# DylanAuty/ObjCAViT

Hardware: AMD Instinct MI355X
Metric: images/sec (640x480, bs=16) forward depth inference, 3 batches of 16 in flight per GPU; AbsRel vs CPU ref (higher is better)
Workload: dtype f32 (fp16 / bf16 split contractions)

## Files before the change

### include/objcavit_hip.h

```cpp
#ifndef OBJCAVIT_HIP_H
#define OBJCAVIT_HIP_H

#include <stddef.h>
#include <stdint.h>

#ifdef __cplusplus
extern "C" {
#endif

typedef void* ocv_stream_t;

#define OCV_ABI_VERSION 5
int ocv_abi_version(void);
const char* ocv_last_error(void);

int ocv_range_flag_set(unsigned* flag);
int ocv_range_flag_take_fwd(unsigned* flag, unsigned* out, ocv_stream_t stream);
int ocv_attention_set_fp32_range(int on);
int ocv_attention_set_dispatch(int form);

#define OCV_ACT_NONE 0
#define OCV_ACT_RELU 1
#define OCV_ACT_LEAKY_RELU 2
#define OCV_ACT_SILU 3
// ... 147 lines not shown
                                    int C, int H, int W, int k, int stride, int pad_t, int pad_l, int Ho, int Wo,
                                    ocv_stream_t stream);
int ocv_se_gate_partials_fwd(const float* part, int tiles, long pixels_per_image, const float* w1, const float* b1,
                             const float* w2t, const float* b2, float* gate, float* hidden_ws, int B, int C, int R,
                             ocv_stream_t stream);
int ocv_depthwise_conv_nhwc_sum_hl_fwd(const float* in, const float* w, const float* bias, float* out, void* out_hl, float* part,
                                       int B, int C, int H, int W, int k, int stride, int pad_t, int pad_l, int Ho, int Wo,
                                       ocv_stream_t stream);
int ocv_se_gate_weights_fwd(const float* part, int tiles, long pixels_per_image, const float* w1, const float* b1,
                            const float* w2t, const float* b2, const float* W, void* w_packed, long w_image_elems, float* gate,
                            float* hidden_ws, int B, int C, int R, int N, ocv_stream_t stream);


size_t ocv_channel_mean_workspace_bytes(int B, int C, long P);
int ocv_channel_mean_nhwc_fwd(const float* x, float* out, int B, int C, long P, void* workspace, size_t workspace_bytes,
                              ocv_stream_t stream);

int ocv_se_gate_fwd(const float* mean, const float* w1, const float* b1, const float* w2t, const float* b2, float* gate,
                    float* hidden_ws, int B, int C, int R, ocv_stream_t stream);

int ocv_conv_nhwc_fwd(const float* x1, int C1, const float* x2, int C2, const void* w_hi, const void* w_lo,
                      const float* bias, const float* residual, float* y, int B, int H, int W, int Cout, int ksize,
                      int act, ocv_stream_t stream);
int ocv_conv_nhwc_exact_fwd(const float* x1, int C1, const float* x2, int C2, const float* w_tap_major, const float* bias,
                            const float* residual, float* y, int B, int H, int W, int Cout, int ksize, int act,
                            ocv_stream_t stream);
int ocv_conv3x3_nhwc_strided_fwd(const float* x, int Cin, const void* w_hi, const void* w_lo, const float* bias,
                                 const float* residual, float* y, int B, int H, int W, int Cout, int stride, int pad_t,
                                 int pad_l, int Ho, int Wo, int act, ocv_stream_t stream);

int ocv_mbconv_expand_dw_tiles(int Ho, int Wo, int k, int stride);
int ocv_mbconv_expand_dw_fwd(const float* x, const void* w_packed, const float* bias_expand, const float* w_dw,
                             const float* bias_dw, float* y, float* part, int B, int H, int W, int Cin, int mid, int k,
                             int stride, int pad_t, int pad_l, int Ho, int Wo, ocv_stream_t stream);

size_t ocv_split_act_elems(int B, int H, int W, int C);

int ocv_conv_nhwc_split_fwd(const void* x_hl, int Cin, const void* w_hi, const void* w_lo, const float* bias,
                            const float* residual, float* y, void* y_hl, int B, int H, int W, int Cout, int ksize,
                            int act, ocv_stream_t stream);
size_t ocv_conv_nhwc_split_workspace_bytes(int B, int H, int W, int Cin, int Cout, int ksize);
int ocv_conv_nhwc_split_ws_fwd(const void* x_hl, int Cin, const void* w_hi, const void* w_lo, const float* bias,
                               const float* residual, float* y, void* y_hl, int B, int H, int W, int Cout, int ksize,
                               int act, void* workspace, size_t workspace_bytes, ocv_stream_t stream);
int ocv_conv_nhwc_split_x_fwd(const void* x_hl, int Cin, const void* w_hi, const void* w_lo, const float* oscale, int f16,
                              const float* bias, const float* residual, float* y, void* y_hl, int B, int H, int W, int Cout,
                              int ksize, int act, void* workspace, size_t workspace_bytes, ocv_stream_t stream);

int ocv_conv3x3_packed_taps_k(int Cin);
int ocv_conv3x3_split_packed_taps_fwd(const void* x_hl, int Cin, const void* w_hi, const void* w_lo, const float* oscale, int f16,
                                      const float* bias, const float* residual, float* y, void* y_hl, int B, int H, int W, int Cout,
                                      int act, ocv_stream_t stream);

size_t ocv_conv3x3_winograd43_workspace_bytes(int B, int H, int W, int Cin, int Cout);
int ocv_conv3x3_winograd43_split_fwd(const void* x_hl, int Cin, const void* u_hi, const void* u_lo, const float* fscale,
                                     const float* cscale, const float* bias, float* y, void* y_hl, int B, int H, int W, int Cout,
                                     int act, int hl_f16, void* workspace, size_t workspace_bytes, ocv_stream_t stream);

int ocv_tap_interp_supported(int h, int w, int H, int W, int Cout);
int ocv_tap_interp_staging_rounds(int h, int w, int H, int W);
int ocv_tap_interp_combine_fwd(const float* z, int h, int w, int zpad, const float* zborder, const float* s, const float* bias,
                               float* y, void* y_hl, int B, int H, int W, int Cout, int act, ocv_stream_t stream);
int ocv_tap_interp_combine_x_fwd(const float* z, int h, int w, int zpad, const float* zborder, const float* s, const float* bias,
                                 float* y, void* y_hl, int hl_f16, int B, int H, int W, int Cout, int act, ocv_stream_t stream);


int ocv_upsample_concat_split_fwd(const float* x, int h, int w, int C1, const float* skip, int C2, void* out_hl, int B,
                                  int H, int W, ocv_stream_t stream);
int ocv_upsample_concat_split_x_fwd(const float* x, int h, int w, int C1, const float* skip, int C2, void* out_hl, int f16, int B,
                                    int H, int W, ocv_stream_t stream);

size_t ocv_depth_metrics_workspace_bytes(int B, int H, int W);
int ocv_depth_metrics_fwd(const float* pred, const float* pred_mirror, int h, int w, const float* gt, int H, int W,
                          float min_depth, float max_depth, int crop_y0, int crop_y1, int crop_x0, int crop_x1,
                          long first_image_id, float* records, int B, void* workspace, size_t workspace_bytes,
                          ocv_stream_t stream);
size_t ocv_depth_metrics_loss_workspace_bytes(int B, int H, int W, int n_bins);
int ocv_depth_metrics_loss_fwd(const float* pred, const float* pred_mirror, int h, int w, const float* gt, int H, int W,
                               float min_depth, float max_depth, int crop_y0, int crop_y1, int crop_x0, int crop_x1,
                               const float* bin_edges, int n_bins, long first_image_id, float* records, float* loss_records, int B,
                               void* workspace, size_t workspace_bytes, ocv_stream_t stream);

int ocv_frame_ingest_fwd(const uint8_t* frames, long frame_stride, long row_stride, int Hs, int Ws, int top, int left,
                         const float* table, float* out, int B, int H, int W, int mirror_too, long mirror_offset,
                         ocv_stream_t stream);
int ocv_depth_ingest_fwd(const uint16_t* depth, long frame_stride, long row_stride, int Hs, int Ws, int top, int left, float factor,
                         float* out, int B, int H, int W, ocv_stream_t stream);
int ocv_depth_finalize_fwd(const float* pred, const float* pred_mirror, int h, int w, float min_depth, float max_depth, int H, int W,
                           float* depth, uint16_t* depth_u16, float u16_scale, uint8_t* rgb8, const uint8_t* colormap, float vmin,
                           float colormap_scale, int B, ocv_stream_t stream);
int ocv_depth_finalize_stats_fwd(const float* pred, const float* pred_mirror, const float* var, const float* var_mirror,
                                 const float* pmax, const float* pmax_mirror, int h, int w, float min_depth, float max_depth, int H, int W,
                                 float* depth_std, float* confidence, int B, ocv_stream_t stream);
int ocv_object_depth_fwd(const float* depth, const float* depth_std, const float* xywh, long xywh_row_stride, const int* counts, int B,
                         int cap, int H, int W, float half, const double* quantiles, int Q, float* out, ocv_stream_t stream);
#define OCV_UNPROJECT_TILE 2048
size_t ocv_depth_unproject_workspace_bytes(int B, int H, int W, int sy, int sx);
int ocv_depth_unproject_fwd(const float* depth, const float* K, const float* confidence, const float* depth_std, const uint8_t* frames,
                            long frame_stride, long row_stride, int Hs, int Ws, int top, int left, int B, int H, int W, int sy, int sx,
                            float near, float far, float min_confidence, float max_std, int cap, float* points, int* pixel, int* counts,
                            int* total, void* workspace, size_t workspace_bytes, ocv_stream_t stream);

#define OCV_BINNORM_LINEAR 0
#define OCV_BINNORM_SIGMOID 1
#define OCV_BINNORM_NONE 2
int ocv_bin_edges_fwd(const float* raw, int mode, float min_depth, float max_depth, float* widths_normed, float* edges,
// ... 23 lines not shown
```

### objcavit_amd/_lib.py

```python
from __future__ import annotations

import ctypes as C
import os
from typing import Optional

_HERE = os.path.dirname(os.path.abspath(__file__))
LIB_PATH = os.environ.get("OCV_LIB_PATH") or os.path.join(_HERE, "lib", "libobjcavit_hip.so")

_f32p = C.c_void_p
_u8p = C.c_void_p
_stream = C.c_void_p
ABI_VERSION = 5


class EncoderLayerParams(C.Structure):
    _fields_ = [("struct_size", C.c_size_t)] + [(n, C.c_void_p) for n in (
        "in_proj_w", "in_proj_b", "out_proj_w", "out_proj_b", "norm1_w", "norm1_b",
        "linear1_w", "linear1_b", "linear2_w", "linear2_b", "norm2_w", "norm2_b",
        "in_proj_p3", "out_proj_p3", "linear1_p3", "linear2_p3",
        "in_proj_h2", "out_proj_h2", "linear1_h2", "linear2_h2")]

    def __init__(self, *a, **kw):
        super().__init__(*a, **kw)
        self.struct_size = C.sizeof(EncoderLayerParams)
# ... 84 lines not shown
    "ocv_depth_metrics_workspace_bytes": (C.c_size_t, [C.c_int] * 3),
    "ocv_depth_metrics_fwd": (C.c_int, [_f32p, _f32p, C.c_int, C.c_int, _f32p, C.c_int, C.c_int, C.c_float, C.c_float] + [C.c_int] * 4 +
                              [C.c_long, _f32p, C.c_int, C.c_void_p, C.c_size_t, _stream]),
    "ocv_depth_metrics_loss_workspace_bytes": (C.c_size_t, [C.c_int] * 4),
    "ocv_depth_metrics_loss_fwd": (C.c_int, [_f32p, _f32p, C.c_int, C.c_int, _f32p, C.c_int, C.c_int, C.c_float, C.c_float] + [C.c_int] * 4 +
                                   [_f32p, C.c_int, C.c_long, _f32p, _f32p, C.c_int, C.c_void_p, C.c_size_t, _stream]),
    "ocv_frame_ingest_fwd": (C.c_int, [_u8p, C.c_long, C.c_long, C.c_int, C.c_int, C.c_int, C.c_int, _f32p, _f32p, C.c_int, C.c_int, C.c_int,
                                       C.c_int, C.c_long, _stream]),
    "ocv_depth_ingest_fwd": (C.c_int, [C.c_void_p, C.c_long, C.c_long, C.c_int, C.c_int, C.c_int, C.c_int, C.c_float, _f32p, C.c_int, C.c_int,
                                       C.c_int, _stream]),
    "ocv_depth_finalize_fwd": (C.c_int, [_f32p, _f32p, C.c_int, C.c_int, C.c_float, C.c_float, C.c_int, C.c_int, _f32p, C.c_void_p, C.c_float,
                                         _u8p, _u8p, C.c_float, C.c_float, C.c_int, _stream]),
    "ocv_depth_finalize_stats_fwd": (C.c_int, [_f32p] * 6 + [C.c_int, C.c_int, C.c_float, C.c_float, C.c_int, C.c_int, _f32p, _f32p, C.c_int,
                                               _stream]),
    "ocv_object_depth_fwd": (C.c_int, [_f32p, _f32p, _f32p, C.c_long, C.c_void_p, C.c_int, C.c_int, C.c_int, C.c_int, C.c_float,
                                       C.POINTER(C.c_double), C.c_int, _f32p, _stream]),
    "ocv_depth_unproject_workspace_bytes": (C.c_size_t, [C.c_int] * 5),
    "ocv_depth_unproject_fwd": (C.c_int, [_f32p, _f32p, _f32p, _f32p, _u8p, C.c_long, C.c_long] + [C.c_int] * 9 + [C.c_float] * 4 +
                                [C.c_int, _f32p, C.c_void_p, C.c_void_p, C.c_void_p, C.c_void_p, C.c_size_t, _stream]),
    "ocv_conv3x3_few_channels_fwd": (C.c_int, [_f32p, C.c_long, C.c_long, C.c_long, C.c_long, _f32p, _f32p] + [C.c_int] * 5 + [_stream]),
    "ocv_stem_conv_fwd": (C.c_int, [_f32p, _f32p, _f32p, _f32p] + [C.c_int] * 12 + [_stream]),
    "ocv_pointwise_packed_weight_elems": (C.c_size_t, [C.c_int, C.c_int]),
    "ocv_pointwise_split_set_dispatch": (C.c_int, [C.c_int, C.c_int, C.c_int]),
    "ocv_pointwise_conv_nhwc_split_fwd": (C.c_int, [_f32p, _f32p, C.c_int, C.c_void_p, _f32p, _f32p, _f32p,
                                                    C.c_long, C.c_int, C.c_int, C.c_int, C.c_void_p]),
    "ocv_pointwise_conv_nhwc_fwd": (C.c_int, [_f32p, _f32p, C.c_int, _f32p, _f32p, _f32p, _f32p, C.c_long, C.c_int, C.c_int,
                                              C.c_int, _stream]),
    "ocv_depthwise_conv_nhwc_fwd": (C.c_int, [_f32p, _f32p, _f32p, _f32p] + [C.c_int] * 11 + [_stream]),
    "ocv_channel_mean_workspace_bytes": (C.c_size_t, [C.c_int, C.c_int, C.c_long]),
    "ocv_channel_mean_nhwc_fwd": (C.c_int, [_f32p, _f32p, C.c_int, C.c_int, C.c_long, C.c_void_p, C.c_size_t, _stream]),
    "ocv_se_gate_fwd": (C.c_int, [_f32p] * 7 + [C.c_int] * 3 + [_stream]),
    "ocv_conv_nhwc_fwd": (C.c_int, [_f32p, C.c_int, _f32p, C.c_int, C.c_void_p, C.c_void_p, _f32p, _f32p, _f32p] +
                          [C.c_int] * 6 + [_stream]),
    "ocv_conv3x3_nhwc_strided_fwd": (C.c_int, [_f32p, C.c_int, C.c_void_p, C.c_void_p, _f32p, _f32p, _f32p] + [C.c_int] * 10 + [_stream]),
    "ocv_conv_nhwc_exact_fwd": (C.c_int, [_f32p, C.c_int, _f32p, C.c_int, _f32p, _f32p, _f32p, _f32p] + [C.c_int] * 6 + [_stream]),
    "ocv_mbconv_expand_dw_tiles": (C.c_int, [C.c_int] * 4),
    "ocv_mbconv_expand_dw_fwd": (C.c_int, [_f32p, C.c_void_p, _f32p, _f32p, _f32p, _f32p, _f32p] + [C.c_int] * 11 + [_stream]),
    "ocv_regressor_bins_fwd": (C.c_int, [_f32p, C.c_long, _f32p, _f32p, _f32p, _f32p, _f32p, _f32p, C.c_int, C.c_int, C.c_int, C.c_int, C.c_float,
                                         C.c_int, C.c_float, C.c_float, _f32p, _f32p, _f32p, C.c_int, _stream]),
    "ocv_bin_edges_fwd": (C.c_int, [_f32p, C.c_int, C.c_float, C.c_float, _f32p, _f32p, _f32p, C.c_int, C.c_int, _stream]),
    "ocv_object_tokens_pad_fwd": (C.c_int, [_f32p, C.c_void_p, C.c_float, _f32p, _u8p, C.c_int, C.c_int, C.c_int, _stream]),
    "ocv_object_front_pad_fwd": (C.c_int, [_f32p, C.c_void_p, C.c_int, C.c_int, C.c_float, _f32p, _u8p] + [C.c_int] * 4 + [_stream]),
    "ocv_split_act_elems": (C.c_size_t, [C.c_int] * 4),
    "ocv_conv_nhwc_split_fwd": (C.c_int, [C.c_void_p, C.c_int, C.c_void_p, C.c_void_p, _f32p, _f32p, _f32p, C.c_void_p]
                                + [C.c_int] * 6 + [_stream]),
    "ocv_conv_nhwc_split_workspace_bytes": (C.c_size_t, [C.c_int] * 6),
    "ocv_conv_nhwc_split_ws_fwd": (C.c_int, [C.c_void_p, C.c_int, C.c_void_p, C.c_void_p, _f32p, _f32p, _f32p, C.c_void_p]
                                   + [C.c_int] * 6 + [C.c_void_p, C.c_size_t, _stream]),
    "ocv_conv_nhwc_split_x_fwd": (C.c_int, [C.c_void_p, C.c_int, C.c_void_p, C.c_void_p, _f32p, C.c_int, _f32p, _f32p, _f32p, C.c_void_p]
                                  + [C.c_int] * 6 + [C.c_void_p, C.c_size_t, _stream]),
    "ocv_conv3x3_packed_taps_k": (C.c_int, [C.c_int]),
    "ocv_conv3x3_split_packed_taps_fwd": (C.c_int, [C.c_void_p, C.c_int, C.c_void_p, C.c_void_p, _f32p, C.c_int, _f32p, _f32p, _f32p, C.c_void_p]
                                          + [C.c_int] * 5 + [_stream]),
    "ocv_upsample_concat_split_x_fwd": (C.c_int, [_f32p, C.c_int, C.c_int, C.c_int, _f32p, C.c_int, C.c_void_p, C.c_int,
                                                  C.c_int, C.c_int, C.c_int, _stream]),
    "ocv_tap_interp_combine_x_fwd": (C.c_int, [_f32p, C.c_int, C.c_int, C.c_int, _f32p, _f32p, _f32p, _f32p, C.c_void_p] + [C.c_int] * 6 + [_stream]),
    "ocv_pos_grid_sample_fwd": (C.c_int, [_f32p, C.c_int, C.c_int, C.c_int, _f32p, C.c_int, C.c_int, C.c_int, C.c_float, C.c_float,
                                          C.c_int, _f32p, _f32p, _stream]),
    "ocv_conv3x3_winograd43_workspace_bytes": (C.c_size_t, [C.c_int] * 5),
    "ocv_conv3x3_winograd43_split_fwd": (C.c_int, [C.c_void_p, C.c_int, C.c_void_p, C.c_void_p, _f32p, _f32p, _f32p, _f32p, C.c_void_p] + [C.c_int] * 6 +
                                         [C.c_void_p, C.c_size_t, _stream]),
    "ocv_tap_interp_supported": (C.c_int, [C.c_int] * 5),
    "ocv_tap_interp_staging_rounds": (C.c_int, [C.c_int] * 4),
    "ocv_tap_interp_combine_fwd": (C.c_int, [_f32p, C.c_int, C.c_int, C.c_int, _f32p, _f32p, _f32p, _f32p, C.c_void_p] + [C.c_int] * 5 + [_stream]),
    "ocv_upsample_concat_split_fwd": (C.c_int, [_f32p, C.c_int, C.c_int, C.c_int, _f32p, C.c_int, C.c_void_p,
                                                C.c_int, C.c_int, C.c_int, _stream]),
}

_lib: Optional[C.CDLL] = None


class HipLibraryError(RuntimeError):
    pass


def load(path: Optional[str] = None) -> C.CDLL:
    global _lib
    if _lib is not None and path is None:
        return _lib
    import torch
    p = path or LIB_PATH
    if not os.path.exists(p):
        raise HipLibraryError(
            f"{p} not found: build it with `python -m objcavit_amd.build` (hipcc --offload-arch=gfx950). "
            "There is no CPU fallback for the ObjCAViT hot path.")
    try:
        lib = C.CDLL(p, mode=C.RTLD_GLOBAL)
    except OSError as e:
        raise HipLibraryError(f"cannot load {p}: {e}") from e
    for name, (res, args) in PROTOTYPES.items():
        try:
            fn = getattr(lib, name)
        except AttributeError as e:
            raise HipLibraryError(f"{p} does not export {name}") from e
        fn.restype = res
        fn.argtypes = args
    if lib.ocv_abi_version() != ABI_VERSION:
        raise HipLibraryError(f"ABI version mismatch: library {lib.ocv_abi_version()}, binding {ABI_VERSION}")
    if path is None:
        _lib = lib
    return lib


def check(rc: int, what: str) -> None:
    if rc != 0:
        msg = load().ocv_last_error().decode(errors="replace")
# ... 2 lines not shown
```

### objcavit_amd/build.py

```python
from __future__ import annotations

import os
import shutil
import subprocess
import sys

HERE = os.path.dirname(os.path.abspath(__file__))
CSRC = os.environ.get("OCV_CSRC_DIR") or os.path.join(HERE, "csrc")
LIB_DIR = os.path.join(HERE, "lib")
LIB_PATH = os.path.join(LIB_DIR, "libobjcavit_hip.so")
SOURCES = ("capi.hip", "linear.hip", "attention.hip", "patch_embed.hip", "bin_head.hip", "depthwise.hip", "conv_igemm.hip", "encoder_nhwc.hip", "upsample.hip", "pointwise_split.hip", "stem.hip", "depthwise_se.hip", "metrics.hip", "mbconv_fused.hip", "pos_sample.hip", "conv_exact.hip", "token_split3.hip", "tap_interp.hip", "pointwise_hl.hip", "xattn_h2.hip", "conv_few.hip", "token_h2.hip", "objects_pad.hip", "bin_edges.hip", "frame_ingest.hip", "depth_finalize.hip", "object_depth.hip", "point_cloud.hip")
ARCH = "gfx950"


def _hipcc() -> str:
    for c in (os.environ.get("HIPCC"), shutil.which("hipcc"), "/opt/rocm/bin/hipcc"):
        if c and os.path.exists(c):
            return c
    raise RuntimeError("hipcc not found")


def _stale() -> bool:
    if not os.path.exists(LIB_PATH):
        return True
    t = os.path.getmtime(LIB_PATH)
    deps = [os.path.join(CSRC, f) for f in os.listdir(CSRC)] + [os.path.join(HERE, "..", "include", "objcavit_hip.h")]
    return any(os.path.getmtime(d) > t for d in deps)


def build(force: bool = False, verbose: bool = False, out: str = None) -> str:
    out = out or os.environ.get("OCV_LIB_OUT")
    if out:
        return _build_to(os.path.abspath(out), os.path.abspath(out) + ".objs", verbose)
    if not force and not _stale():
        return LIB_PATH
    return _build_to(LIB_PATH, LIB_DIR, verbose)


def _build_to(lib_path: str, obj_dir: str, verbose: bool) -> str:
    os.makedirs(os.path.dirname(lib_path), exist_ok=True)
    os.makedirs(obj_dir, exist_ok=True)
    if os.path.exists(lib_path):
        os.remove(lib_path)
    objs = []
    procs = []
    for src in SOURCES:
        obj = os.path.join(obj_dir, src.replace(".hip", ".o"))
        cmd = [_hipcc(), f"--offload-arch={ARCH}", "-O3", "-std=c++17", "-fPIC", "-ffp-contract=fast", "-c",
               os.path.join(CSRC, src), "-o", obj] + os.environ.get("OCV_EXTRA_HIPCC_FLAGS", "").split()
        if verbose:
            cmd.insert(1, "-Rpass-analysis=kernel-resource-usage")
        procs.append((src, subprocess.Popen(cmd, stdout=subprocess.PIPE, stderr=subprocess.STDOUT, text=True)))
        objs.append(obj)
    for src, pr in procs:
        out, _ = pr.communicate()
        if pr.returncode != 0:
            raise RuntimeError(f"hipcc failed on {src}:\n{out}")
        if verbose:
            print(out)
    link = [_hipcc(), f"--offload-arch={ARCH}", "-shared", "-fPIC", "-o", lib_path] + objs
    r = subprocess.run(link, stdout=subprocess.PIPE, stderr=subprocess.STDOUT, text=True)
    if r.returncode != 0:
        raise RuntimeError(f"link failed:\n{r.stdout}")
    for o in objs:
# ... 9 lines not shown
```

### objcavit_amd/csrc/common.hpp

```cpp
#pragma once
#include <hip/hip_runtime.h>
#include <stdint.h>

typedef float f32x16 __attribute__((ext_vector_type(16)));
typedef float f32x4 __attribute__((ext_vector_type(4)));

#define OCV_WAVE 64

__device__ __forceinline__ f32x16 mfma_32x32x2(float a, float b, f32x16 c) {
  return __builtin_amdgcn_mfma_f32_32x32x2f32(a, b, c, 0, 0, 0);
}

__device__ __forceinline__ constexpr int acc_row(int r, int hh) { return (r & 3) + 8 * (r >> 2) + 4 * hh; }

__device__ __forceinline__ float wave_sum(float v) {
#pragma unroll
  for (int o = 32; o > 0; o >>= 1) v += __shfl_xor(v, o, 64);
  return v;
}

__device__ __forceinline__ float xor32_max(float v) { return fmaxf(v, __shfl_xor(v, 32, 64)); }
__device__ __forceinline__ float xor32_sum(float v) { return v + __shfl_xor(v, 32, 64); }

__device__ __forceinline__ float fast_exp(float x) { return __builtin_amdgcn_exp2f(x * 1.44269504088896340736f); }
// ... 20 lines not shown
__device__ __forceinline__ void ocv_range_note(unsigned* flag, float amax) {
  if (flag != nullptr && amax > OCV_F16_GUARD) atomicOr(flag, 1u);
}
__device__ __forceinline__ float ocv_amax4(float m, const f32x4 v) {
  return fmaxf(fmaxf(m, fmaxf(fabsf(v[0]), fabsf(v[1]))), fmaxf(fabsf(v[2]), fabsf(v[3])));
}


typedef __attribute__((address_space(1))) unsigned ocv_gu32;
__device__ __forceinline__ void ocv_store_sc1(float* p, float v) {
  __hip_atomic_store((ocv_gu32*)p, __float_as_uint(v), __ATOMIC_RELAXED, __HIP_MEMORY_SCOPE_AGENT);
}

void ocv_set_error(const char* fmt, ...);

unsigned* ocv_range_flag_current();

#define OCV_CHECK_ARG(cond, ...)        \
  do {                                  \
    if (!(cond)) {                      \
      ocv_set_error(__VA_ARGS__);       \
      return -1;                        \
    }                                   \
  } while (0)

#define OCV_CHECK_LAUNCH(name)                                              \
  do {                                                                      \
    hipError_t e__ = hipGetLastError();                                     \
    if (e__ != hipSuccess) {                                                \
      ocv_set_error("%s: launch failed: %s", name, hipGetErrorString(e__)); \
      return (int)e__;                                                      \
    }                                                                       \
  } while (0)

int ocv_zero_async(void* p, size_t nbytes, hipStream_t stream);

int ocv_attention_launch(const float* q, long q_bs, int q_ss, const float* k, long k_bs, int k_ss, const float* v,
                         long v_bs, int v_ss, const uint8_t* key_padding_mask, int mask_ld, float* ctx, long o_bs,
                         int o_ss, int B, int H, int Sq, int Sk, float scale, hipStream_t stream);

int ocv_cross_attn_fused_launch(const float* q_src, const float* k_src, const float* v_src, const uint8_t* mask, int mask_ld,
                                const float* in_w, const float* in_b, const float* out_w, const float* out_b, float* out, int B,
                                int Sq, int Sk, int Se, int E, int H, hipStream_t st);

int ocv_cross_attn_split3_launch(const float* q_src, const float* k_src, const float* v_src, const uint8_t* mask, int mask_ld,
                                 const void* in_p3, const float* in_b, const void* out_p3, const float* out_b, float* out,
                                 float* kv_ws, int B, int Sq, int Sk, int Se, int E, int H, hipStream_t st);

int ocv_ffn_split_count(int M, int FF);
int ocv_ffn_split_launch(const float* x, const float* w1, const float* b1, const float* w2, const float* b2,
                         const float* gamma, const float* beta, float eps, const uint8_t* zero_row_mask, float* out, int M,
                         int FF, float* part, int nsplit, hipStream_t st);

bool ocv_layer_params_view(const void* caller_params, int index, void* lib_params);

static inline bool ocv_aligned16(const void* p) { return (reinterpret_cast<uintptr_t>(p) & 15) == 0; }
static inline int ocv_cdiv(long a, long b) { return (int)((a + b - 1) / b); }
```

### objcavit_amd/csrc/conv_igemm.hip

```cpp
#include <stdlib.h>

#include "common.hpp"
#include "../../include/objcavit_hip.h"

namespace {

typedef __bf16 bf16x8 __attribute__((ext_vector_type(8)));
typedef _Float16 cv_h16x8 __attribute__((ext_vector_type(8)));
typedef _Float16 cv_h16x4 __attribute__((ext_vector_type(4)));
typedef __bf16 ti4 __attribute__((ext_vector_type(4)));

constexpr int CBM = 256, CBN = 128, CBK = 32;
constexpr int ROWB = 80;
constexpr int A_BYTES = CBM * ROWB, B_BYTES = CBN * ROWB;
constexpr int BUF_BYTES = 2 * A_BYTES + 2 * B_BYTES;

struct ConvArgs {
  const float* x1; const float* x2;
  const __bf16* xhl;
  __bf16* yhl;
  int Cpo;
  const __bf16* whi; const __bf16* wlo;
  const float* bias; const float* res; float* y;
  int C1, C2, Cin, Cp, Cout, H, W, ks, act;
// ... 705 lines not shown
  a.whi = (const __bf16*)w_hi; a.wlo = (const __bf16*)w_lo; a.bias = bias; a.res = residual; a.y = y;
  a.C1 = Cin; a.C2 = 0; a.Cin = Cin; a.Cout = Cout; a.H = H; a.W = W; a.ks = ksize; a.act = act; a.ksplit = 1;
  a.f16 = f16; a.oscale = oscale;
  a.range_flag = (f16 && y_hl != nullptr) ? ocv_range_flag_current() : nullptr;
  if (y_hl != nullptr && Cout % 32 != 0) {
    const int zrc = ocv_zero_async(y_hl, ocv_split_act_elems(B, H, W, Cout) * sizeof(__bf16), (hipStream_t)stream);
    if (zrc != 0) return zrc;
  }
  const long M = (long)B * H * W;
  const int ks = conv_ksplit(M, Cout, Cin, ksize);
  if (ks > 1 && workspace != nullptr && workspace_bytes >= (size_t)ks * M * Cout * sizeof(float)) {
    ConvArgs h = a;
    h.bias = nullptr; h.res = nullptr; h.yhl = nullptr; h.act = OCV_ACT_NONE; h.y = (float*)workspace; h.ksplit = ks; h.oscale = nullptr;
    const int rc = launch_conv(h, B, (hipStream_t)stream);
    if (rc != 0) return rc;
    FinArgs f{(const float*)workspace, bias, residual, y, (__bf16*)y_hl, M, M * Cout / 8, Cout, a.Cpo, act, ks, oscale, f16, a.range_flag};
    hipLaunchKernelGGL(conv_splitk_finish_kernel, dim3((unsigned)((f.items + 255) / 256)), dim3(256), 0, (hipStream_t)stream, f);
    OCV_CHECK_LAUNCH("ocv_conv_nhwc_split_fwd(finish)");
    return 0;
  }
  return launch_conv(a, B, (hipStream_t)stream);
}

extern "C" int ocv_conv3x3_packed_taps_k(int Cin) {
  if (Cin < 1 || Cin > 2040) return 0;
  const int gpt = (Cin + 7) / 8;
  return (9 * gpt + 3) / 4 * CBK;
}

extern "C" int ocv_conv3x3_split_packed_taps_fwd(const void* x_hl, int Cin, const void* w_hi, const void* w_lo, const float* oscale,
                                                 int f16, const float* bias, const float* residual, float* y, void* y_hl, int B,
                                                 int H, int W, int Cout, int act, ocv_stream_t stream) {
  OCV_CHECK_ARG(x_hl && w_hi && w_lo && (y || y_hl), "ocv_conv3x3_split_packed_taps_fwd: null pointer");
  OCV_CHECK_ARG(ocv_aligned16(y) && ocv_aligned16(y_hl) && ocv_aligned16(residual), "ocv_conv3x3_split_packed_taps_fwd: outputs and residual must be 16-byte aligned");
  OCV_CHECK_ARG(B >= 1 && H >= 1 && W >= 1 && Cout >= 1 && Cin >= 8 && Cin % 8 == 0 && Cin <= 2040,
                "ocv_conv3x3_split_packed_taps_fwd: bad sizes (Cin must be a multiple of 8 in [8, 2040], got %d)", Cin);
  OCV_CHECK_ARG(act >= 0 && act <= 3, "ocv_conv3x3_split_packed_taps_fwd: unknown activation %d", act);
  OCV_CHECK_ARG(f16 == 0 || f16 == 1, "ocv_conv3x3_split_packed_taps_fwd: f16 must be 0 (bf16 pairs) or 1 (fp16 pairs)");
  OCV_CHECK_ARG((reinterpret_cast<uintptr_t>(x_hl) & 127) == 0 && ocv_aligned16(w_hi) && ocv_aligned16(w_lo),
                "ocv_conv3x3_split_packed_taps_fwd: x_hl must be 128-byte aligned, weights 16-byte aligned");
  const int Kp = ocv_conv3x3_packed_taps_k(Cin), gpt = Cin / 8;
  OCV_CHECK_ARG((long)B * H * W * (Cin + 32) * 4 < (1L << 32) && (long)Cout * Kp * 2 < (1L << 32),
                "ocv_conv3x3_split_packed_taps_fwd: each operand must be smaller than 4 GiB");
  const int inv = (65536 + gpt - 1) / gpt;
  for (int G = 0; G < Kp / 8; ++G)
    OCV_CHECK_ARG((int)(((unsigned)G * (unsigned)inv) >> 16) == G / gpt, "ocv_conv3x3_split_packed_taps_fwd: internal (reciprocal of %d inexact at %d)", gpt, G);
  ConvArgs a{};
  a.xhl = (const __bf16*)x_hl; a.yhl = (__bf16*)y_hl; a.Cpo = (Cout + 31) / 32 * 32;
  a.whi = (const __bf16*)w_hi; a.wlo = (const __bf16*)w_lo; a.bias = bias; a.res = residual; a.y = y;
  a.C1 = Cin; a.C2 = 0; a.Cin = Cin; a.Cout = Cout; a.H = H; a.W = W; a.ks = 3; a.act = act; a.ksplit = 1;
  a.f16 = f16; a.oscale = oscale;
  a.gpt = gpt; a.gpt_inv = inv; a.Kp = Kp;
  a.range_flag = (f16 && y_hl != nullptr) ? ocv_range_flag_current() : nullptr;
  if (y_hl != nullptr && Cout % 32 != 0) {
    const int zrc = ocv_zero_async(y_hl, ocv_split_act_elems(B, H, W, Cout) * sizeof(__bf16), (hipStream_t)stream);
    if (zrc != 0) return zrc;
  }
  return launch_conv(a, B, (hipStream_t)stream);
}

extern "C" int ocv_conv_nhwc_split_ws_fwd(const void* x_hl, int Cin, const void* w_hi, const void* w_lo, const float* bias,
                                          const float* residual, float* y, void* y_hl, int B, int H, int W, int Cout,
                                          int ksize, int act, void* workspace, size_t workspace_bytes, ocv_stream_t stream) {
  return ocv_conv_nhwc_split_x_fwd(x_hl, Cin, w_hi, w_lo, nullptr, 0, bias, residual, y, y_hl, B, H, W, Cout, ksize, act, workspace,
                                   workspace_bytes, stream);
}

extern "C" int ocv_conv_nhwc_split_fwd(const void* x_hl, int Cin, const void* w_hi, const void* w_lo, const float* bias,
                                       const float* residual, float* y, void* y_hl, int B, int H, int W, int Cout,
                                       int ksize, int act, ocv_stream_t stream) {
  return ocv_conv_nhwc_split_ws_fwd(x_hl, Cin, w_hi, w_lo, bias, residual, y, y_hl, B, H, W, Cout, ksize, act, nullptr, 0, stream);
}

extern "C" int ocv_conv_nhwc_fwd(const float* x1, int C1, const float* x2, int C2, const void* w_hi, const void* w_lo,
                                 const float* bias, const float* residual, float* y, int B, int H, int W, int Cout,
                                 int ksize, int act, ocv_stream_t stream) {
  OCV_CHECK_ARG(x1 && w_hi && w_lo && y, "ocv_conv_nhwc_fwd: null pointer");
  OCV_CHECK_ARG(ksize == 1 || ksize == 3, "ocv_conv_nhwc_fwd: kernel size must be 1 or 3 (got %d)", ksize);
  OCV_CHECK_ARG(B >= 1 && H >= 1 && W >= 1 && Cout >= 1 && C1 >= 4, "ocv_conv_nhwc_fwd: bad sizes");
  OCV_CHECK_ARG(C1 % 4 == 0 && (x2 == nullptr || (C2 >= 4 && C2 % 4 == 0 && C1 % CBK == 0)),
                "ocv_conv_nhwc_fwd: channel counts must be multiples of 4 (and C1 a multiple of %d when a second tensor is concatenated)", CBK);
  OCV_CHECK_ARG(act >= 0 && act <= 3, "ocv_conv_nhwc_fwd: unknown activation %d", act);
  OCV_CHECK_ARG(ocv_aligned16(x1) && ocv_aligned16(x2) && ocv_aligned16(w_hi) && ocv_aligned16(w_lo),
                "ocv_conv_nhwc_fwd: operands must be 16-byte aligned");
  OCV_CHECK_ARG((long)B * H * W * C1 * 4 < (1L << 32) && (long)B * H * W * (x2 ? C2 : 0) * 4 < (1L << 32) &&
                    9L * Cout * (C1 + C2 + 32) * 2 < (1L << 32),
                "ocv_conv_nhwc_fwd: each operand must be smaller than 4 GiB (32-bit byte offsets inside the kernel)");
  ConvArgs a{};
  a.x1 = x1; a.x2 = x2; a.whi = (const __bf16*)w_hi; a.wlo = (const __bf16*)w_lo;
  a.bias = bias; a.res = residual; a.y = y;
  a.C1 = C1; a.C2 = x2 ? C2 : 0; a.Cin = a.C1 + a.C2;
  a.Cout = Cout; a.H = H; a.W = W; a.act = act;
  a.Ho = H; a.Wo = W; a.pad_t = a.pad_l = ksize / 2;
  const hipStream_t st = (hipStream_t)stream;
  if (ksize == 1) return x2 ? launch_igemm<1, 1, true>(a, B, st, "ocv_conv_nhwc") : launch_igemm<1, 1, false>(a, B, st, "ocv_conv_nhwc");
  return x2 ? launch_igemm<3, 1, true>(a, B, st, "ocv_conv_nhwc") : launch_igemm<3, 1, false>(a, B, st, "ocv_conv_nhwc");
}

extern "C" int ocv_conv3x3_nhwc_strided_fwd(const float* x, int Cin, const void* w_hi, const void* w_lo, const float* bias,
                                            const float* residual, float* y, int B, int H, int W, int Cout, int stride,
                                            int pad_t, int pad_l, int Ho, int Wo, int act, ocv_stream_t stream) {
  OCV_CHECK_ARG(x && w_hi && w_lo && y, "ocv_conv3x3_nhwc_strided_fwd: null pointer");
  OCV_CHECK_ARG(B >= 1 && H >= 1 && W >= 1 && Ho >= 1 && Wo >= 1 && Cout >= 1 && Cin >= 4 && Cin % 4 == 0,
                "ocv_conv3x3_nhwc_strided_fwd: bad sizes (Cin must be a positive multiple of 4)");
  OCV_CHECK_ARG(stride == 1 || stride == 2, "ocv_conv3x3_nhwc_strided_fwd: stride must be 1 or 2 (got %d)", stride);
  OCV_CHECK_ARG(pad_t >= 0 && pad_l >= 0 && pad_t < 3 && pad_l < 3, "ocv_conv3x3_nhwc_strided_fwd: bad padding (%d, %d)", pad_t, pad_l);
// ... 402 lines not shown
```

### objcavit_amd/hip_ops/conv.py

```python
from __future__ import annotations

import ctypes as C
import math
import os
import threading
from typing import Dict, Optional, Sequence, Tuple

import torch

from .. import _lib
from .._lib import EncoderLayerParams, check
from ._core import *


class SplitAct:
    __slots__ = ("hl", "C")

    def __init__(self, hl: torch.Tensor, C: int):
        self.hl, self.C = hl, int(C)

    @staticmethod
    def empty(B: int, C: int, H: int, W: int, device, f16: bool = False) -> "SplitAct":
        Cp = (C + 31) // 32 * 32
        n = int(_lib.load().ocv_split_act_elems(B, H, W, C))
# ... 95 lines not shown
    col = col[col > 0]
    return bool(col.numel() == 0 or float(col.min()) >= 2.0 ** -17)


def prep_conv_weight(weight: torch.Tensor, f16: bool = False):
    Cout, Cin, kh, kw = weight.shape
    if kh != kw or kh not in (1, 3):
        raise ValueError("prep_conv_weight: kernel must be 1x1 or 3x3")
    w = weight.detach().float().permute(2, 3, 0, 1).reshape(kh * kw, Cout, Cin)
    Cp = (Cin + 31) // 32 * 32
    if not f16:
        if Cp != Cin:
            w = torch.nn.functional.pad(w, (0, Cp - Cin))
        hi = w.to(torch.bfloat16)
        lo = (w - hi.float()).to(torch.bfloat16)
        return hi.contiguous(), lo.contiguous()
    amax = w.abs().amax(dim=(0, 2))
    k = torch.where(amax > 0, torch.round(8.0 - torch.log2(amax.clamp_min(1e-30))), torch.zeros_like(amax)).clamp(-100.0, 100.0)
    w = w * torch.exp2(k)[None, :, None]
    if Cp != Cin:
        w = torch.nn.functional.pad(w, (0, Cp - Cin))
    hi = w.to(torch.float16)
    lo = (w - hi.float()).to(torch.float16)
    return hi.contiguous(), lo.contiguous(), torch.exp2(-k).float().contiguous()


def packed_taps_pay(Cin: int) -> bool:
    if Cin < 8 or Cin % 8 != 0:
        return False
    packed = (9 * (Cin // 8) + 3) // 4
    dense = 9 * ((Cin + 31) // 32)
    return 6 * packed <= 5 * dense


def prep_conv_weight_packed_taps(weight: torch.Tensor, f16: bool = False):
    Cout, Cin, kh, kw = weight.shape
    if (kh, kw) != (3, 3) or Cin % 8 != 0:
        raise ValueError("prep_conv_weight_packed_taps: needs a 3x3 kernel over a multiple of 8 input channels")
    Kp = int(_lib.load().ocv_conv3x3_packed_taps_k(Cin))
    w = weight.detach().float().permute(0, 2, 3, 1).reshape(Cout, 9 * Cin)
    w = torch.nn.functional.pad(w, (0, Kp - 9 * Cin)).reshape(1, Cout, Kp)
    if not f16:
        hi = w.to(torch.bfloat16)
        lo = (w - hi.float()).to(torch.bfloat16)
        return hi.contiguous(), lo.contiguous()
    amax = w.abs().amax(dim=(0, 2))
    k = torch.where(amax > 0, torch.round(8.0 - torch.log2(amax.clamp_min(1e-30))), torch.zeros_like(amax)).clamp(-100.0, 100.0)
    w = w * torch.exp2(k)[None, :, None]
    hi = w.to(torch.float16)
    lo = (w - hi.float()).to(torch.float16)
    return hi.contiguous(), lo.contiguous(), torch.exp2(-k).float().contiguous()


def conv3x3_split_packed_taps(x: SplitAct, w_hi: torch.Tensor, w_lo: torch.Tensor, bias: Optional[torch.Tensor], act: int = ACT_NONE,
                              out_fp32: bool = True, out_split: bool = False, oscale: Optional[torch.Tensor] = None):
    lib = _lib.load()
    if not (out_fp32 or out_split):
        raise ValueError("conv3x3_split_packed_taps: nothing to output")
    dt = x.hl.dtype
    _req(x.hl, "x.hl", dt)
    B, Cin, H, W = x.shape
    if x.hl.dim() != 4 or x.hl.shape[3] != 2 * ((Cin + 31) // 32 * 32):
        raise ValueError("conv3x3_split_packed_taps: x.hl must be [B, H, W, 2 * ceil32(C)]")
    for n, t in (("w_hi", w_hi), ("w_lo", w_lo)):
        _req(t, n, dt)
    Kp = int(lib.ocv_conv3x3_packed_taps_k(Cin))
    if Cin % 8 != 0 or Kp == 0 or w_hi.dim() != 3 or w_hi.shape[0] != 1 or w_hi.shape[2] != Kp or w_lo.shape != w_hi.shape:
        raise ValueError(f"conv3x3_split_packed_taps: weights {tuple(w_hi.shape)} do not match {Cin} input channels (Kp = {Kp})")
    Cout = w_hi.shape[1]
    for n, t in (("bias", bias), ("oscale", oscale)):
        if t is not None:
            _req(t, n)
            if t.numel() != Cout:
                raise ValueError(f"conv3x3_split_packed_taps: {n} size mismatch")
    y = torch.empty(B, Cout, H, W, dtype=torch.float32, device=x.hl.device, memory_format=torch.channels_last) if out_fp32 else None
    ys = SplitAct.empty(B, Cout, H, W, x.hl.device, f16=x.f16) if out_split else None
    ptrs = (x.hl.data_ptr(), Cin, w_hi.data_ptr(), w_lo.data_ptr(), _ptr(oscale), int(x.f16), _ptr(bias), None, _ptr(y),
            ys.hl.data_ptr() if out_split else None, B, H, W, Cout, act)
    keep = (x, w_hi, w_lo, oscale, bias, y, ys)
    launch(f"conv3x3p|{B},{H},{W},{Cin},{Cout}",
           lambda: (keep, check(lib.ocv_conv3x3_split_packed_taps_fwd(*ptrs, _stream()), "ocv_conv3x3_split_packed_taps_fwd"))[1])
    _note_range(f"conv3x3p|{B},{H},{W},{Cin},{Cout}", ys)
    if out_fp32 and out_split:
        return y, ys
    return y if out_fp32 else ys


def conv_nhwc_exact(x1: torch.Tensor, x2: Optional[torch.Tensor], w_tap_major: torch.Tensor, bias: Optional[torch.Tensor],
                    ksize: int, act: int = ACT_NONE, residual: Optional[torch.Tensor] = None) -> torch.Tensor:
    lib = _lib.load()
    x1 = _nhwc(x1, "x1")
    B, C1, H, W = x1.shape
    C2 = 0
    if x2 is not None:
        x2 = _nhwc(x2, "x2")
        if x2.shape[0] != B or x2.shape[2:] != x1.shape[2:]:
            raise ValueError("conv_nhwc_exact: x2 must match x1 in batch and spatial size")
        C2 = x2.shape[1]
    _req(w_tap_major, "w_tap_major")
    if w_tap_major.dim() != 3 or w_tap_major.shape[0] != ksize * ksize or w_tap_major.shape[2] != C1 + C2:
        raise ValueError(f"conv_nhwc_exact: weights {tuple(w_tap_major.shape)} do not match {C1}+{C2} input channels, k={ksize}")
    Cout = w_tap_major.shape[1]
    if bias is not None:
        _req(bias, "bias")
        if bias.numel() != Cout:
            raise ValueError("conv_nhwc_exact: bias size mismatch")
    y = torch.empty(B, Cout, H, W, dtype=torch.float32, device=x1.device, memory_format=torch.channels_last)
    if residual is not None:
        residual = _nhwc(residual, "residual")
# ... 236 lines not shown
```

Measured before the change: 1084.

## Add persistent weight-stationary streaming kernel for packed-tap 3x3 skip convs

Adds a new kernel for packed-tap 3x3 convolutions with Cin 24 or 40 whose output is plain fp32, with no bias, activation or residual. It keeps the hi/lo weight fragments in registers for the whole kernel. Each workgroup walks a contiguous run of spatial tiles and double-buffers halo loads into LDS via global_load_lds, so the next tile's load overlaps the current tile's MFMA work. Workgroups are mapped across the XCDs. By default it is used only for the two shapes listed as faster (24->128 and 40->256); an environment variable can force it on or off. The risks are high register pressure, fixed per-shape configuration, and a Python env check added to every call.

```diff
diff --git a/include/objcavit_hip.h b/include/objcavit_hip.h
--- a/include/objcavit_hip.h
+++ b/include/objcavit_hip.h
@@ -223,6 +223,9 @@
                                       const float* bias, const float* residual, float* y, void* y_hl, int B, int H, int W, int Cout,
                                       int act, ocv_stream_t stream);
 
+int ocv_conv_skip_stream_set_dispatch(int mode);
+int ocv_conv_skip_stream_plan(int B, int H, int W, int Cin, int Cout, int f16, int* workgroups, int* tiles);
+
 size_t ocv_conv3x3_winograd43_workspace_bytes(int B, int H, int W, int Cin, int Cout);
 int ocv_conv3x3_winograd43_split_fwd(const void* x_hl, int Cin, const void* u_hi, const void* u_lo, const float* fscale,
                                      const float* cscale, const float* bias, float* y, void* y_hl, int B, int H, int W, int Cout,
diff --git a/objcavit_amd/_lib.py b/objcavit_amd/_lib.py
--- a/objcavit_amd/_lib.py
+++ b/objcavit_amd/_lib.py
@@ -160,6 +160,8 @@
     "ocv_conv3x3_packed_taps_k": (C.c_int, [C.c_int]),
     "ocv_conv3x3_split_packed_taps_fwd": (C.c_int, [C.c_void_p, C.c_int, C.c_void_p, C.c_void_p, _f32p, C.c_int, _f32p, _f32p, _f32p, C.c_void_p]
                                           + [C.c_int] * 5 + [_stream]),
+    "ocv_conv_skip_stream_set_dispatch": (C.c_int, [C.c_int]),
+    "ocv_conv_skip_stream_plan": (C.c_int, [C.c_int] * 6 + [C.POINTER(C.c_int), C.POINTER(C.c_int)]),
     "ocv_upsample_concat_split_x_fwd": (C.c_int, [_f32p, C.c_int, C.c_int, C.c_int, _f32p, C.c_int, C.c_void_p, C.c_int,
                                                   C.c_int, C.c_int, C.c_int, _stream]),
     "ocv_tap_interp_combine_x_fwd": (C.c_int, [_f32p, C.c_int, C.c_int, C.c_int, _f32p, _f32p, _f32p, _f32p, C.c_void_p] + [C.c_int] * 6 + [_stream]),
diff --git a/objcavit_amd/build.py b/objcavit_amd/build.py
--- a/objcavit_amd/build.py
+++ b/objcavit_amd/build.py
@@ -9,7 +9,7 @@
 CSRC = os.environ.get("OCV_CSRC_DIR") or os.path.join(HERE, "csrc")
 LIB_DIR = os.path.join(HERE, "lib")
 LIB_PATH = os.path.join(LIB_DIR, "libobjcavit_hip.so")
-SOURCES = ("capi.hip", "linear.hip", "attention.hip", "patch_embed.hip", "bin_head.hip", "depthwise.hip", "conv_igemm.hip", "encoder_nhwc.hip", "upsample.hip", "pointwise_split.hip", "stem.hip", "depthwise_se.hip", "metrics.hip", "mbconv_fused.hip", "pos_sample.hip", "conv_exact.hip", "token_split3.hip", "tap_interp.hip", "pointwise_hl.hip", "xattn_h2.hip", "conv_few.hip", "token_h2.hip", "objects_pad.hip", "bin_edges.hip", "frame_ingest.hip", "depth_finalize.hip", "object_depth.hip", "point_cloud.hip")
+SOURCES = ("capi.hip", "linear.hip", "attention.hip", "patch_embed.hip", "bin_head.hip", "depthwise.hip", "conv_igemm.hip", "encoder_nhwc.hip", "upsample.hip", "pointwise_split.hip", "stem.hip", "depthwise_se.hip", "metrics.hip", "mbconv_fused.hip", "pos_sample.hip", "conv_exact.hip", "token_split3.hip", "tap_interp.hip", "pointwise_hl.hip", "xattn_h2.hip", "conv_few.hip", "token_h2.hip", "objects_pad.hip", "bin_edges.hip", "frame_ingest.hip", "depth_finalize.hip", "object_depth.hip", "point_cloud.hip", "conv_skip_stream.hip")
 ARCH = "gfx950"
 
 
diff --git a/objcavit_amd/csrc/common.hpp b/objcavit_amd/csrc/common.hpp
--- a/objcavit_amd/csrc/common.hpp
+++ b/objcavit_amd/csrc/common.hpp
@@ -96,6 +96,10 @@
                          const float* gamma, const float* beta, float eps, const uint8_t* zero_row_mask, float* out, int M,
                          int FF, float* part, int nsplit, hipStream_t st);
 
+bool ocv_skip_stream_takes(int Cin, int Cout, int f16);
+int ocv_skip_stream_launch(const void* x_hl, int Cin, const void* w_hi, const void* w_lo, const float* oscale, int f16, float* y, int B,
+                           int H, int W, int Cout, int Kp, hipStream_t stream);
+
 bool ocv_layer_params_view(const void* caller_params, int index, void* lib_params);
 
 static inline bool ocv_aligned16(const void* p) { return (reinterpret_cast<uintptr_t>(p) & 15) == 0; }
diff --git a/objcavit_amd/csrc/conv_igemm.hip b/objcavit_amd/csrc/conv_igemm.hip
--- a/objcavit_amd/csrc/conv_igemm.hip
+++ b/objcavit_amd/csrc/conv_igemm.hip
@@ -781,6 +781,8 @@
   a.f16 = f16; a.oscale = oscale;
   a.gpt = gpt; a.gpt_inv = inv; a.Kp = Kp;
   a.range_flag = (f16 && y_hl != nullptr) ? ocv_range_flag_current() : nullptr;
+  if (y_hl == nullptr && bias == nullptr && residual == nullptr && act == OCV_ACT_NONE && ocv_skip_stream_takes(Cin, Cout, f16))
+    return ocv_skip_stream_launch(x_hl, Cin, w_hi, w_lo, oscale, f16, y, B, H, W, Cout, Kp, (hipStream_t)stream);
   if (y_hl != nullptr && Cout % 32 != 0) {
     const int zrc = ocv_zero_async(y_hl, ocv_split_act_elems(B, H, W, Cout) * sizeof(__bf16), (hipStream_t)stream);
     if (zrc != 0) return zrc;
diff --git a/objcavit_amd/csrc/conv_skip_stream.hip b/objcavit_amd/csrc/conv_skip_stream.hip
--- /dev/null
+++ b/objcavit_amd/csrc/conv_skip_stream.hip
@@ -0,0 +1,283 @@
+#include "common.hpp"
+#include "../../include/objcavit_hip.h"
+
+namespace {
+
+typedef __bf16 ss_bf16x8 __attribute__((ext_vector_type(8)));
+typedef _Float16 ss_h16x8 __attribute__((ext_vector_type(8)));
+typedef __attribute__((address_space(1))) const void* ss_gptr;
+typedef __attribute__((address_space(3))) void* ss_lptr;
+
+__device__ __attribute__((aligned(256))) float ss_zero_page[64];
+
+struct SSArgs {
+  const char* x;
+  const char* whi; const char* wlo;
+  const float* oscale;
+  float* y;
+  int H, W, Cout, Kp;
+  int tiles_x, tiles_y, ntiles;
+  int nruns, ncb;
+};
+
+template <int GPT>
+struct SSCfg {
+  static constexpr int KS = (9 * GPT + 3) / 4;
+  static constexpr int NSL = GPT <= 3 ? 2 : 1;
+  static constexpr int TY = 8, TX = GPT <= 3 ? 32 : 16;
+  static constexpr int HX = TX + 2, HY = TY + 2;
+  static constexpr int CH = 2 * GPT;
+  static constexpr int NC = HX * HY * CH;
+  static constexpr int NR = (NC + 255) / 256;
+  static constexpr int BUF = NR * 256 * 16;
+  static constexpr int CBLK = 4 * NSL * 16;
+  static constexpr int PIXB = (GPT + 3) / 4 * 128;
+  static constexpr int GX = TX / 16;
+  static constexpr int NPG = TY * GX, PG = 4;
+  static_assert(NC + 2 * GPT <= NR * 256, "zero chunks for the K padding behind the halo");
+  static_assert(2 * BUF <= 80 * 1024, "at most half of the CU's LDS");
+  static_assert(NPG % PG == 0, "whole batches");
+};
+
+__device__ __forceinline__ void ss_drain_vm() {
+  __builtin_amdgcn_s_waitcnt((7 << 4) | (15 << 8));
+  asm volatile("" ::: "memory");
+}
+__device__ __forceinline__ void ss_barrier() {
+  asm volatile("" ::: "memory");
+  __builtin_amdgcn_s_barrier();
+  asm volatile("" ::: "memory");
+}
+
+template <bool F16>
+__device__ __forceinline__ f32x4 ss_mfma(const ss_bf16x8 a, const ss_bf16x8 b, const f32x4 c) {
+  if constexpr (F16) return __builtin_amdgcn_mfma_f32_16x16x32_f16(__builtin_bit_cast(ss_h16x8, a), __builtin_bit_cast(ss_h16x8, b), c, 0, 0, 0);
+  else return __builtin_amdgcn_mfma_f32_16x16x32_bf16(a, b, c, 0, 0, 0);
+}
+
+template <int GPT, bool F16>
+__global__ __launch_bounds__(256, 2) void conv_skip_stream_kernel(SSArgs p) {
+  using C = SSCfg<GPT>;
+  extern __shared__ __attribute__((aligned(1024))) unsigned char lds[];
+
+  const int tid = threadIdx.x, lane = tid & 63;
+  const int wave = __builtin_amdgcn_readfirstlane(tid >> 6);
+  const int l15 = lane & 15, q4 = lane >> 4;
+
+  int run, cb;
+  {
+    const int wg = blockIdx.x, xcd = wg & 7, idx = wg >> 3;
+    cb = idx % p.ncb;
+    run = xcd * (p.nruns >> 3) + idx / p.ncb;
+  }
+  const int t0 = (int)((long)p.ntiles * run / p.nruns), t1 = (int)((long)p.ntiles * (run + 1) / p.nruns);
+  if (t0 >= t1) return;
+  const int n0 = cb * C::CBLK + wave * (C::NSL * 16);
+
+  ss_bf16x8 wh[C::NSL][C::KS], wl[C::NSL][C::KS];
+  float sv[C::NSL][4];
+#pragma unroll
+  for (int sl = 0; sl < C::NSL; ++sl) {
+    const long wo = ((long)(n0 + 16 * sl + l15) * p.Kp + 8 * q4) * 2;
+#pragma unroll
+    for (int s = 0; s < C::KS; ++s) {
+      wh[sl][s] = *reinterpret_cast<const ss_bf16x8*>(p.whi + wo + 64 * s);
+      wl[sl][s] = *reinterpret_cast<const ss_bf16x8*>(p.wlo + wo + 64 * s);
+    }
+#pragma unroll
+    for (int r = 0; r < 4; ++r) sv[sl][r] = p.oscale != nullptr ? p.oscale[n0 + 16 * sl + 4 * q4 + r] : 1.f;
+  }
+
+  int koff[C::KS];
+#pragma unroll
+  for (int s = 0; s < C::KS; ++s) {
+    const int G = 4 * s + q4;
+    const int tap = G / GPT, cg = G - tap * GPT;
+    const int ky = tap / 3, kx = tap - 3 * ky;
+    koff[s] = tap < 9 ? ((ky * C::HX + kx) * C::CH + cg) * 16 : -1;
+  }
+
+  auto tile_origin = [&](int t, int& b, int& Y0, int& X0) {
+    const int tx = t % p.tiles_x, r = t / p.tiles_x;
+    const int ty = r % p.tiles_y;
+    b = r / p.tiles_y;
+    Y0 = ty * C::TY;
+    X0 = tx * C::TX;
+  };
+
+  auto issue_halo = [&](int t, int buf) {
+    int b, Y0, X0;
+    tile_origin(t, b, Y0, X0);
+    const unsigned img = (unsigned)b * (unsigned)p.H;
+#pragma unroll
+    for (int r = 0; r < C::NR; ++r) {
+      const int c = r * 256 + tid;
+      const int pix = c / C::CH, part = c - pix * C::CH;
+      const int hy = pix / C::HX, hx = pix - hy * C::HX;
+      const int Y = Y0 - 1 + hy, X = X0 - 1 + hx;
+      const bool ok = c < C::NC && (unsigned)Y < (unsigned)p.H && (unsigned)X < (unsigned)p.W;
+      const int g = part < GPT ? part : part - GPT;
+      const unsigned poff = (unsigned)((g >> 2) * 128 + (g & 3) * 16 + (part < GPT ? 0 : 64));
+      const unsigned off = ((img + (unsigned)Y) * (unsigned)p.W + (unsigned)X) * (unsigned)C::PIXB + poff;
+      const void* src = ok ? (const void*)(p.x + off) : (const void*)ss_zero_page;
+      unsigned char* dst = lds + buf * C::BUF + (r * 256 + wave * 64) * 16;
+      __builtin_amdgcn_global_load_lds((ss_gptr)src, (ss_lptr)dst, 16, 0, 0);
+    }
+  };
+
+  issue_halo(t0, 0);
+  ss_drain_vm();
+  for (int t = t0; t < t1; ++t) {
+    const int buf = (t - t0) & 1;
+    ss_barrier();
+    if (t + 1 < t1) issue_halo(t + 1, buf ^ 1);
+    int b, Y0, X0;
+    tile_origin(t, b, Y0, X0);
+    const unsigned char* hb = lds + buf * C::BUF;
+    const int zoff = C::NC * 16;
+    float* yb = p.y + n0 + 4 * q4;
+
+    for (int bt = 0; bt < C::NPG / C::PG; ++bt) {
+      if (Y0 + (bt * C::PG) / C::GX >= p.H) {
+        if (bt == 0) ss_drain_vm();
+        break;
+      }
+      int pbase[C::PG];
+#pragma unroll
+      for (int g = 0; g < C::PG; ++g) {
+        const int pg = bt * C::PG + g, ry = pg / C::GX, cx = pg - ry * C::GX;
+        pbase[g] = ((ry * C::HX + cx * 16 + l15) * C::CH) * 16;
+      }
+      f32x4 acc[C::NSL][C::PG];
+#pragma unroll
+      for (int sl = 0; sl < C::NSL; ++sl)
+#pragma unroll
+        for (int g = 0; g < C::PG; ++g) acc[sl][g] = f32x4{0.f, 0.f, 0.f, 0.f};
+
+#pragma unroll
+      for (int s = 0; s < C::KS; ++s) {
+        ss_bf16x8 xh[C::PG], xl[C::PG];
+#pragma unroll
+        for (int g = 0; g < C::PG; ++g) {
+          const int a = (s == C::KS - 1 && koff[s] < 0) ? zoff : pbase[g] + koff[s];
+          xh[g] = *reinterpret_cast<const ss_bf16x8*>(hb + a);
+          xl[g] = *reinterpret_cast<const ss_bf16x8*>(hb + a + GPT * 16);
+        }
+#pragma unroll
+        for (int sl = 0; sl < C::NSL; ++sl)
+#pragma unroll
+          for (int g = 0; g < C::PG; ++g) acc[sl][g] = ss_mfma<F16>(wh[sl][s], xh[g], acc[sl][g]);
+#pragma unroll
+        for (int sl = 0; sl < C::NSL; ++sl)
+#pragma unroll
+          for (int g = 0; g < C::PG; ++g) acc[sl][g] = ss_mfma<F16>(wl[sl][s], xh[g], acc[sl][g]);
+#pragma unroll
+        for (int sl = 0; sl < C::NSL; ++sl)
+#pragma unroll
+          for (int g = 0; g < C::PG; ++g) acc[sl][g] = ss_mfma<F16>(wh[sl][s], xl[g], acc[sl][g]);
+      }
+
+      if (bt == 0) ss_drain_vm();
+#pragma unroll
+      for (int g = 0; g < C::PG; ++g) {
+        const int pg = bt * C::PG + g, ry = pg / C::GX, cx = pg - ry * C::GX;
+        const int Y = Y0 + ry, X = X0 + cx * 16 + l15;
+        if (Y < p.H && X < p.W) {
+          float* o = yb + (((long)b * p.H + Y) * p.W + X) * p.Cout;
+#pragma unroll
+          for (int sl = 0; sl < C::NSL; ++sl) {
+            f32x4 v;
+#pragma unroll
+            for (int r = 0; r < 4; ++r) v[r] = fmaf(acc[sl][g][r], sv[sl][r], 0.f);
+            *reinterpret_cast<f32x4*>(o + 16 * sl) = v;
+          }
+        }
+      }
+    }
+  }
+}
+
+int g_skip_stream_mode = 2;
+
+int ss_gpt(int Cin) { return Cin == 24 ? 3 : Cin == 40 ? 5 : 0; }
+int ss_cblk(int gpt) { return gpt == 3 ? SSCfg<3>::CBLK : SSCfg<5>::CBLK; }
+
+bool ss_covers(int Cin, int Cout) {
+  const int gpt = ss_gpt(Cin);
+  return gpt != 0 && Cout % ss_cblk(gpt) == 0;
+}
+bool ss_measured_faster(int Cin, int Cout, int f16) {
+  (void)f16;
+  return (Cin == 24 && Cout == 128) || (Cin == 40 && Cout == 256);
+}
+
+int ss_cus() {
+  static int cus = 0;
+  if (cus == 0) {
+    int dev = 0, n = 0;
+    if (hipGetDevice(&dev) != hipSuccess || hipDeviceGetAttribute(&n, hipDeviceAttributeMultiprocessorCount, dev) != hipSuccess || n < 8) n = 256;
+    cus = n;
+  }
+  return cus;
+}
+
+void ss_plan(SSArgs& a, int B, int H, int W, int gpt) {
+  const int ty = gpt == 3 ? SSCfg<3>::TY : SSCfg<5>::TY, tx = gpt == 3 ? SSCfg<3>::TX : SSCfg<5>::TX;
+  a.tiles_x = ocv_cdiv(W, tx);
+  a.tiles_y = ocv_cdiv(H, ty);
+  a.ntiles = B * a.tiles_y * a.tiles_x;
+  a.ncb = a.Cout / ss_cblk(gpt);
+  int most = 2 * ss_cus() / a.ncb / 8 * 8;
+  if (most < 8) most = 8;
+  const int per = ocv_cdiv(a.ntiles, most);
+  a.nruns = (ocv_cdiv(a.ntiles, per) + 7) / 8 * 8;
+}
+
+template <int GPT, bool F16>
+int ss_launch(const SSArgs& a, hipStream_t st) {
+  static bool attr = false;
+  if (!attr) {
+    (void)hipFuncSetAttribute((const void*)conv_skip_stream_kernel<GPT, F16>, hipFuncAttributeMaxDynamicSharedMemorySize, 2 * SSCfg<GPT>::BUF);
+    attr = true;
+  }
+  hipLaunchKernelGGL((conv_skip_stream_kernel<GPT, F16>), dim3(a.nruns * a.ncb), dim3(256), 2 * SSCfg<GPT>::BUF, st, a);
+  OCV_CHECK_LAUNCH("ocv_conv3x3_split_packed_taps_fwd(stream)");
+  return 0;
+}
+
+}
+
+bool ocv_skip_stream_takes(int Cin, int Cout, int f16) {
+  if (g_skip_stream_mode == 0 || !ss_covers(Cin, Cout)) return false;
+  return g_skip_stream_mode == 1 || ss_measured_faster(Cin, Cout, f16);
+}
+
+int ocv_skip_stream_launch(const void* x_hl, int Cin, const void* w_hi, const void* w_lo, const float* oscale, int f16, float* y, int B,
+                           int H, int W, int Cout, int Kp, hipStream_t stream) {
+  const int gpt = ss_gpt(Cin);
+  OCV_CHECK_ARG(ss_covers(Cin, Cout) && Kp == SSCfg<3>::KS * 32 * (gpt == 3) + SSCfg<5>::KS * 32 * (gpt == 5),
+                "ocv_conv3x3_split_packed_taps_fwd(stream): internal (shape %d -> %d not covered)", Cin, Cout);
+  OCV_CHECK_ARG((long)B * H * W * Cout < (1L << 40) && (long)B * ocv_cdiv(H, 8) * ocv_cdiv(W, 16) < (1L << 30),
+                "ocv_conv3x3_split_packed_taps_fwd(stream): too many tiles");
+  SSArgs a{(const char*)x_hl, (const char*)w_hi, (const char*)w_lo, oscale, y, H, W, Cout, Kp, 0, 0, 0, 0, 0};
+  ss_plan(a, B, H, W, gpt);
+  if (gpt == 3) return f16 ? ss_launch<3, true>(a, stream) : ss_launch<3, false>(a, stream);
+  return f16 ? ss_launch<5, true>(a, stream) : ss_launch<5, false>(a, stream);
+}
+
+extern "C" int ocv_conv_skip_stream_set_dispatch(int mode) {
+  OCV_CHECK_ARG(mode >= 0 && mode <= 2, "ocv_conv_skip_stream_set_dispatch: mode must be 0 (off), 1 (on) or 2 (auto), got %d", mode);
+  g_skip_stream_mode = mode;
+  return 0;
+}
+
+extern "C" int ocv_conv_skip_stream_plan(int B, int H, int W, int Cin, int Cout, int f16, int* workgroups, int* tiles) {
+  OCV_CHECK_ARG(B >= 1 && H >= 1 && W >= 1 && Cin >= 1 && Cout >= 1, "ocv_conv_skip_stream_plan: bad sizes");
+  if (!ocv_skip_stream_takes(Cin, Cout, f16)) return 0;
+  SSArgs a{};
+  a.Cout = Cout;
+  ss_plan(a, B, H, W, ss_gpt(Cin));
+  if (workgroups != nullptr) *workgroups = a.nruns * a.ncb;
+  if (tiles != nullptr) *tiles = a.ntiles;
+  return 1;
+}
diff --git a/objcavit_amd/hip_ops/conv.py b/objcavit_amd/hip_ops/conv.py
--- a/objcavit_amd/hip_ops/conv.py
+++ b/objcavit_amd/hip_ops/conv.py
@@ -171,9 +171,31 @@
     return hi.contiguous(), lo.contiguous(), torch.exp2(-k).float().contiguous()
 
 
+_SKIP_STREAM_MODES = {"0": 0, "1": 1, "auto": 2}
+_skip_stream_set = [None]
+
+
+def skip_stream_sync() -> None:
+    mode = os.environ.get("OCV_SKIP_STREAM", "auto")
+    if mode != _skip_stream_set[0]:
+        if mode not in _SKIP_STREAM_MODES:
+            raise ValueError(f"OCV_SKIP_STREAM={mode!r}: expected '0', '1' or 'auto' (default)")
+        check(_lib.load().ocv_conv_skip_stream_set_dispatch(_SKIP_STREAM_MODES[mode]), "ocv_conv_skip_stream_set_dispatch")
+        _skip_stream_set[0] = mode
+
+
+def skip_stream_plan(B: int, H: int, W: int, Cin: int, Cout: int, f16: bool):
+    skip_stream_sync()
+    nwg, nt = C.c_int(0), C.c_int(0)
+    rc = _lib.load().ocv_conv_skip_stream_plan(B, H, W, Cin, Cout, int(f16), C.byref(nwg), C.byref(nt))
+    check(min(rc, 0), "ocv_conv_skip_stream_plan")
+    return (nwg.value, nt.value) if rc == 1 else None
+
+
 def conv3x3_split_packed_taps(x: SplitAct, w_hi: torch.Tensor, w_lo: torch.Tensor, bias: Optional[torch.Tensor], act: int = ACT_NONE,
                               out_fp32: bool = True, out_split: bool = False, oscale: Optional[torch.Tensor] = None):
     lib = _lib.load()
+    skip_stream_sync()
     if not (out_fp32 or out_split):
         raise ValueError("conv3x3_split_packed_taps: nothing to output")
     dt = x.hl.dtype
```

Result: no change. 1090, median of 6 (+0.6%).
